# ultravideo/kvazzup

Measured on AMD Instinct MI355X. Metric: hevc_encode_decode_fps, higher is better.
Workload: dtype u8

## Files before the change

### kvazzup_amd/csrc/dec_parse.hip

```cpp
#include <chrono>
#include <cstdio>
#include <cstdlib>
#include <cstring>
#include "decoder.h"

namespace kvzx {

enum { PART_2Nx2N = 0, PART_2NxN, PART_Nx2N, PART_NxN, PART_2NxnU, PART_2NxnD, PART_nLx2N, PART_nRx2N };

namespace {

struct StateTabs { uint8_t next_mps[128], next_lps[128]; uint8_t next[128][2]; uint8_t lps[128][4]; uint32_t lpsn[128][4]; };
const StateTabs &state_tabs()
{
  static const StateTabs t = [] {
    StateTabs t;
    for (int s = 0; s < 128; s++) {
      int st = s >> 1, mps = s & 1;
      t.next_mps[s] = (uint8_t)(((st < 62 ? st + 1 : st) << 1) | mps);
      t.next_lps[s] = (uint8_t)((kNextLps[st] << 1) | (st == 0 ? mps ^ 1 : mps));
      t.next[s][0] = t.next_mps[s]; t.next[s][1] = t.next_lps[s];
      for (int q = 0; q < 4; q++) { t.lps[s][q] = kRangeLps[st][q]; const int n = __builtin_clz((uint32_t)kRangeLps[st][q]) - 23; t.lpsn[s][q] = ((uint32_t)kRangeLps[st][q] << n) | ((uint32_t)n << 16) | ((uint32_t)kRangeLps[st][q] << 24); }
    }
    return t;
  }();
  return t;
}
struct CabacRegs {
  const uint8_t *p = nullptr, *end = nullptr;
  uint64_t value = 0; int bits = 0;
  uint32_t range = 510; uint32_t past = 0;
  const StateTabs *st = nullptr;
  uint16_t *ctx = nullptr;
  static __attribute__((noinline)) uint32_t word_tail(const uint8_t *p, const uint8_t *end) { uint32_t w = 0; for (int i = 0; i < 4; i++) w = (w << 8) | (p + i < end ? p[i] : 0u); return w; }
  __attribute__((always_inline)) inline uint32_t word()
  {
    uint32_t w;
    if (__builtin_expect(p + 4 <= end, 1)) { memcpy(&w, p, 4); w = __builtin_bswap32(w); }
    else { w = word_tail(p, end); past++; }
    p += 4;
    return w;
  }
  __attribute__((always_inline)) inline void refill() { if (__builtin_expect(bits < 16, 0)) { value = (value << 32) | word(); bits += 32; } }
  bool overrun() const { return past > 3; }
  __attribute__((always_inline)) inline int bin(int ci)
  {
    const uint32_t s = ctx[ci];
    const uint32_t e = st->lpsn[s][(range >> 6) & 3];
    const uint32_t rmps = range - (e >> 24);
    const uint64_t scaled = (uint64_t)rmps << bits;
    const bool isl = value >= scaled;
    value -= isl ? scaled : 0;
    const uint32_t nm = (rmps >> 8) ^ 1u;
    range = isl ? (e & 0x1ffu) : (rmps << nm);
    bits -= (int)(isl ? ((e >> 16) & 15u) : nm);
    ctx[ci] = st->next[s][isl];
    refill();
    return (int)((s & 1u) ^ (uint32_t)isl);
  }
  __attribute__((always_inline)) inline int bypass()
  {
    bits--;
    const uint64_t scaled = (uint64_t)range << bits;
    int b = 0;
    if (value >= scaled) { value -= scaled; b = 1; }
    refill();
    return b;
  }
  __attribute__((always_inline)) inline uint32_t bypass_bits(int n)
  {
    uint32_t v = 0;
    while (n > 0) {
      const int m = n > 16 ? 16 : n;
      if (m <= 2) { for (int i = 0; i < m; i++) v = (v << 1) | (uint32_t)bypass(); }
      else {
        bits -= m;
        const uint64_t scaled = (uint64_t)range << bits;
        const uint64_t q = value / scaled;
        value -= q * scaled;
        v = (v << m) | (uint32_t)(q & 0xffffu);
        refill();
      }
      n -= m;
    }
    return v;
  }
  __attribute__((always_inline)) inline int terminate()
  {
    range -= 2;
    if (value >= ((uint64_t)range << bits)) return 1;
    if (range < 256) { range <<= 1; bits--; }
    refill();
    return 0;
  }
};
struct CabacDec : CabacRegs {
  const uint8_t *buf = nullptr;
  uint16_t ctx_store[CTX_COUNT];
  CabacDec() { ctx = ctx_store; }
  CabacDec(const CabacDec &) = delete;
  void load_ctx(const uint8_t *src) { for (int i = 0; i < CTX_COUNT; i++) ctx_store[i] = src[i]; }
  void save_ctx(uint8_t *dst) const { for (int i = 0; i < CTX_COUNT; i++) dst[i] = (uint8_t)ctx_store[i]; }
  void start(const uint8_t *b, size_t l)
  {
    buf = b; p = b; end = b + l; past = 0; st = &state_tabs(); range = 510; ctx = ctx_store;
    value = word(); bits = 32 - 9;
    refill();
  }
  size_t bytes_consumed() const { const size_t consumed_bits = (size_t)(p - buf) * 8 - (size_t)bits; return (consumed_bits + 7) >> 3; }
};

std::atomic<long> g_yields{0};

void parse_sao(CabacDec &c, SaoParams &p, const SaoParams *left, const SaoParams *up, bool luma, bool chroma)
{
  memset(&p, 0, sizeof(p));
  if (left && c.bin(CTX_SAO_MERGE)) { p = *left; return; }
  if (up && c.bin(CTX_SAO_MERGE)) { p = *up; return; }
  for (int ci = 0; ci < 3; ci++) {
    if (!(ci ? chroma : luma)) continue;
    if (ci < 2) p.type[ci] = (uint8_t)(c.bin(CTX_SAO_TYPE) ? (c.bypass() ? 2 : 1) : 0);
    else { p.type[2] = p.type[1]; p.eo_class[2] = p.eo_class[1]; }
    if (!p.type[ci]) continue;
    int a[4];
    for (int i = 0; i < 4; i++) { a[i] = 0; while (a[i] < 7 && c.bypass()) a[i]++; }
    if (p.type[ci] == 1) {
      for (int i = 0; i < 4; i++) if (a[i] && c.bypass()) a[i] = -a[i];
      p.band_pos[ci] = (uint8_t)c.bypass_bits(5);
    } else {
      if (ci < 2) p.eo_class[ci] = (uint8_t)c.bypass_bits(2);
      a[2] = -a[2]; a[3] = -a[3];
    }
    for (int i = 0; i < 4; i++) p.offset[ci][i] = (int8_t)a[i];
  }
}

__attribute__((noinline)) uint32_t sig_flag_run(CabacRegs &cr, const uint8_t *pk, int base, int k0)
{
  CabacRegs c = cr;
  uint32_t sig = 0;
  for (int k = k0; k >= 1; k--) sig |= (uint32_t)c.bin(base + pk[k]) << k;
  cr.p = c.p; cr.value = c.value; cr.bits = c.bits; cr.range = c.range; cr.past = c.past;
  return sig;
}
__attribute__((noinline)) uint32_t greater1_run(CabacRegs &cr, int ctx_base, int n, int *c1_io)
{
  CabacRegs c = cr;
  uint32_t g = 0; int c1 = *c1_io;
  for (int j = 0; j < n; j++) {
    const int g1 = c.bin(ctx_base + c1);
    g |= (uint32_t)g1 << j;
    if (g1) c1 = 0; else if (c1 > 0 && c1 < 3) c1++;
  }
  *c1_io = c1;
  cr.p = c.p; cr.value = c.value; cr.bits = c.bits; cr.range = c.range; cr.past = c.past;
  return g;
}

__attribute__((always_inline)) inline bool parse_residual_regs(CabacRegs &c, int log2, int cidx, int scan_idx, bool sign_hiding, bool ts_enabled, int *tskip, std::vector<uint32_t> &out)
{
  const ScanTabs &S = scan_tabs();
  const int n = 1 << log2, sbl = log2 - 2, nsb = 1 << sbl;
  const uint8_t *SX = S.x[scan_idx][sbl], *SY = S.y[scan_idx][sbl], *PX = S.x[scan_idx][2], *PY = S.y[scan_idx][2];
  uint8_t csbf[8][8]; memset(csbf, 0, sizeof(csbf));
  *tskip = (ts_enabled && log2 == 2) ? c.bin(CTX_TS_FLAG + (cidx ? 1 : 0)) : 0;
  int pre[2];
  for (int d = 0; d < 2; d++) {
    int off, sh, mx = (log2 << 1) - 1, v = 0;
    if (cidx == 0) { off = 3 * (log2 - 2) + ((log2 - 1) >> 2); sh = (log2 + 1) >> 2; } else { off = 15; sh = log2 - 2; }
    while (v < mx && c.bin((d ? CTX_LAST_Y : CTX_LAST_X) + off + (v >> sh))) v++;
    pre[d] = v;
  }
  int lx = pre[0], ly = pre[1];
  if (lx > 3) { int nb = (lx >> 1) - 1; lx = (1 << nb) * (2 + (lx & 1)) + (int)c.bypass_bits(nb); }
  if (ly > 3) { int nb = (ly >> 1) - 1; ly = (1 << nb) * (2 + (ly & 1)) + (int)c.bypass_bits(nb); }
  if (scan_idx == 2) { int tt = lx; lx = ly; ly = tt; }
  if (lx >= n || ly >= n) return false;
  const int last_sb = S.inv[scan_idx][sbl][((ly >> 2) << sbl) | (lx >> 2)], last_pos = S.inv[scan_idx][2][((ly & 3) << 2) | (lx & 3)];
  int c1 = 1;
  for (int i = last_sb; i >= 0; i--) {
    const int xs = SX[i], ys = SY[i];
    int right = (xs < nsb - 1) ? csbf[ys][xs + 1] : 0, below = (ys < nsb - 1) ? csbf[ys + 1][xs] : 0, infer_dc = 0;
    if (i < last_sb && i > 0) { csbf[ys][xs] = (uint8_t)c.bin(CTX_CSBF + ((right | below) ? 1 : 0) + (cidx ? 2 : 0)); infer_dc = 1; }
    else csbf[ys][xs] = 1;
    if (!csbf[ys][xs]) continue;
    uint32_t sig = 0;
    if (i == last_sb) sig |= 1u << last_pos;
    const int prev_csbf = right | (below << 1);
    const uint8_t *pk = S.sigk[scan_idx][log2 == 2 ? 4 : prev_csbf];
    const int sig_base = CTX_SIG + (cidx ? 27 : 0);
    const int sig_off = log2 == 2 ? 0 : (cidx == 0 ? ((i > 0 ? 3 : 0) + ((log2 == 3) ? ((scan_idx == 0) ? 9 : 15) : 21)) : ((log2 == 3) ? 9 : 12));
    {
      const int k0 = (i == last_sb) ? last_pos - 1 : 15;
      const int base = sig_base + sig_off;
      if (k0 >= 1) sig |= sig_flag_run(c, pk, base, k0);
      if (k0 >= 0) {
        if (infer_dc && !(sig >> 1)) sig |= 1u;
        else sig |= (uint32_t)c.bin((i == 0 && log2 != 2) ? sig_base : base + pk[0]);
      }
    }
    if (!sig) continue;
    int ctx_set = (i > 0 && cidx == 0) ? 2 : 0;
    if (c1 == 0) ctx_set++;
    c1 = 1;
    int pos[16], lev[16], nsig = 0, g1idx = -1;
    for (uint32_t m = sig; m;) { const int k = 31 - __builtin_clz(m); pos[nsig++] = k; m &= ~(1u << k); }
    for (int j = 0; j < nsig; j++) lev[j] = 1;
    {
      const uint32_t g = greater1_run(c, CTX_GT1 + (cidx ? 16 : 0) + ctx_set * 4, nsig < 8 ? nsig : 8, &c1);
      if (g) { g1idx = __builtin_ctz(g); for (uint32_t m = g; m; m &= m - 1) lev[__builtin_ctz(m)] = 2; }
    }
    if (g1idx >= 0 && c.bin(CTX_GT2 + (cidx ? 4 : 0) + ctx_set)) lev[g1idx] = 3;
    const bool hidden = sign_hiding && (pos[0] - pos[nsig - 1] > 3);
    const int nsigns = hidden ? nsig - 1 : nsig;
    uint32_t signs = c.bypass_bits(nsigns) << (nsig - nsigns);
    int rice = 0, sum = 0;
    for (int j = 0; j < nsig; j++) {
      int base = (j < 8) ? ((j == g1idx) ? 3 : 2) : 1;
      if (lev[j] == base) {
        int prefix = 0;
        while (prefix < 32 && c.bypass()) prefix++;
        if (prefix - 3 + rice > 16) return false;
        int rem = prefix <= 3 ? (prefix << rice) + (int)c.bypass_bits(rice)
                              : (((1 << (prefix - 3)) + 3 - 1) << rice) + (int)c.bypass_bits(prefix - 3 + rice);
        lev[j] = base + rem;
        if (lev[j] > 3 * (1 << rice)) rice = imin(rice + 1, 4);
      }
      sum += lev[j];
    }
    if (hidden && (sum & 1)) signs |= 1u;
    const size_t o0 = out.size();
    out.resize(o0 + (size_t)nsig);
    uint32_t *dst = out.data() + o0;
    for (int j = 0; j < nsig; j++) {
      const int v = ((signs >> (nsig - 1 - j)) & 1) ? -lev[j] : lev[j];
      const int xp = PX[pos[j]], yp = PY[pos[j]];
      dst[j] = (uint32_t)((((ys << 2) + yp) * n + (xs << 2) + xp) << 16) | ((uint32_t)clip3(-32768, 32767, v) & 0xffffu);
    }
    if (c.overrun()) return false;
  }
  return !c.overrun();
}

bool parse_residual(CabacDec &cd, int log2, int cidx, int scan_idx, bool sign_hiding, bool ts_enabled, int *tskip, std::vector<uint32_t> &out)
{
  CabacRegs c = cd;
  const bool ok = parse_residual_regs(c, log2, cidx, scan_idx, sign_hiding, ts_enabled, tskip, out);
  static_cast<CabacRegs &>(cd) = c;
  return ok;
}

struct MvCand { int mvx, mvy, ref_idx; };

struct SliceParser {
  Decoder::PicJob &job; Decoder::SubOut &out;
  const DecSps &sps; const DecPps &pps; const SliceHdr &sh;
  CabacDec c;
  const int w, h, b4w, b8w, ctbl, mincb, wc, hc;
  B4Rec *b4; uint8_t *pm, *ctd, *im;
  int ref_y0 = -(1 << 30), ref_y1 = 1 << 30;
  int tile_y0 = 0, tile_y1 = 1 << 30, tile_x0 = 0, tile_x1 = 1 << 30;
  const uint8_t *slice_of = nullptr; int cur_slice = 0;
  int slice_qp = 26;
  int err = 0;
  int qp_y = 0, qp_y_pred = 0, last_qp_y = 0, cu_qp_delta_val = 0, log2_qg = 6; bool qp_delta_coded = false;
  int cu_pred_mode = 0, part_mode = 0, max_trafo_depth = 0, intra_modes[4] = {0, 0, 0, 0}, chroma_mode = 0; bool intra_split = false;
  uint32_t ctu_intra_mask = 0;

  SliceParser(Decoder::PicJob &j, Decoder::SubOut &o, int pw)
      : job(j), out(o), sps(*j.sps), pps(j.pps), sh(j.sh), w(j.sps->width), h(j.sps->height), b4w(pw / 4), b8w(pw / 8), ctbl(j.sps->ctb_log2), mincb(j.sps->min_cb_log2), wc(j.sps->wc()),
        hc(j.sps->hc()), b4(j.b4), pm(j.pred_mode.data()), ctd(j.ct_depth.data()), im(j.intra_mode.data())
  { log2_qg = ctbl - pps.qp_delta_depth; }

  inline int bi(int x, int y) const { return (y >> 2) * b4w + (x >> 2); }
  inline int b8(int x, int y) const { return (y >> 3) * b8w + (x >> 3); }
  inline bool avail(int, int, int xn, int yn) const
  {
    return xn >= tile_x0 && yn >= tile_y0 && xn < w && yn < h && yn < tile_y1 && xn < tile_x1 && pm[b8(xn, yn)] != PM_NONE && (!slice_of || slice_of[(yn >> ctbl) * wc + (xn >> ctbl)] == cur_slice);
  }
  void fill_cu8(uint8_t *arr, int x0, int y0, int n, int v)
  {
    const int cols = imin(n, w - x0) >> 3;
    for (int y = y0; y < y0 + n && y < h; y += 8) memset(arr + b8(x0, y), v, (size_t)cols);
  }
  void fill_u8(uint8_t *arr, int x0, int y0, int bw, int bh, int v)
  {
    const int cols = imin(bw, w - x0) >> 2;
    for (int y = y0; y < y0 + bh && y < h; y += 4) memset(arr + bi(x0, y), v, (size_t)cols);
  }
  bool cu_edges_done = false;
  int cu_bypass = 0;
  void fill_recs(int x0, int y0, int bw, int bh, const B4Rec &r, bool cu_edges = false)
  {
    uint64_t v; memcpy(&v, &r, 8);
    const int cols = imin(bw, w - x0) >> 2;
    if (!cu_edges) { for (int y = y0; y < y0 + bh && y < h; y += 4) { uint64_t *p = (uint64_t *)&b4[bi(x0, y)]; for (int i = 0; i < cols; i++) p[i] = v; } return; }
    B4Rec e = r;
    e.flags |= B4_EDGE_V | B4_TU_V; uint64_t vl; memcpy(&vl, &e, 8);
    e.flags = r.flags | B4_EDGE_H | B4_TU_H; uint64_t vt; memcpy(&vt, &e, 8);
    e.flags |= B4_EDGE_V | B4_TU_V; uint64_t vc; memcpy(&vc, &e, 8);
    for (int y = y0; y < y0 + bh && y < h; y += 4) {
      uint64_t *p = (uint64_t *)&b4[bi(x0, y)];
      const bool top = y == y0;
      if (cols > 0) p[0] = top ? vc : vl;
      for (int i = 1; i < cols; i++) p[i] = top ? vt : v;
    }
    cu_edges_done = true;
  }
  void emit_tu(const DecTu &td)
  {
    const int X = td.plane ? td.x * 2 : td.x, Y = td.plane ? td.y * 2 : td.y;
    if (ctbl == 6) {
      TuRange &r = job.region[(Y >> 5) * (b4w >> 3) + (X >> 5)];
      if (!r.count) r.first = (uint32_t)out.tus.size();
      r.count++;
    }
    out.tus.push_back(td);
  }

  bool pb_avail(int xcb, int ycb, int ncbs, int xpb, int ypb, int npbw, int npbh, int part_idx, int xn, int yn) const
  {
    const bool same_cb = xcb <= xn && ycb <= yn && xcb + ncbs > xn && ycb + ncbs > yn;
    bool a;
    if (!same_cb) a = avail(xpb, ypb, xn, yn);
    else a = !((npbw << 1) == ncbs && (npbh << 1) == ncbs && part_idx == 1 && (ycb + npbh <= yn) && (xcb + npbw > xn));
    if (a && pm[b8(xn, yn)] == PM_INTRA) a = false;
    return a;
  }
  static bool same_motion(const B4Rec &a, const B4Rec &b) { return a.ref_idx == b.ref_idx && a.mvx == b.mvx && a.mvy == b.mvy; }

  inline int list_poc(int L, int idx) const { return L ? job.ref_poc1[idx & 15] : job.ref_poc[idx & 15]; }
  inline bool list_lt(int L, int idx) const { return (L ? job.ref_lt1[idx & 15] : job.ref_lt[idx & 15]) != 0; }
  static void scale_by(int &mvx, int &mvy, int td_, int tb_)
  {
    const int td = clip3(-128, 127, td_), tb = clip3(-128, 127, tb_);
    if (td == 0) return;
    const int tx = (16384 + (iabs(td) >> 1)) / td, dsf = clip3(-4096, 4095, (tb * tx + 32) >> 6);
    const int px = dsf * mvx, py = dsf * mvy;
    mvx = clip3(-32768, 32767, (px < 0 ? -1 : 1) * ((iabs(px) + 127) >> 8));
    mvy = clip3(-32768, 32767, (py < 0 ? -1 : 1) * ((iabs(py) + 127) >> 8));
  }
  bool temporal_mv(int xpb, int ypb, int npbw, int npbh, int X, int ref_idx, int &mvx, int &mvy)
  {
    ColMotion *col = job.col.get();
    if (!col) return false;
    const int cy = ypb >> ctbl;
    if (cy < col->hc) {
      std::atomic<uint8_t> &d = col->row_done[(size_t)cy];
      int spins = 0;
      while (!d.load(std::memory_order_acquire)) { if (++spins < 2000) __builtin_ia32_pause(); else std::this_thread::yield(); }
    }
    const int cand[2][2] = {{xpb + npbw, ypb + npbh}, {xpb + (npbw >> 1), ypb + (npbh >> 1)}};
    for (int k = 0; k < 2; k++) {
      int x = cand[k][0], y = cand[k][1];
      if (k == 0 && !((ypb >> ctbl) == (y >> ctbl) && y < h && x < w)) continue;
      x >>= 4; y >>= 4;
      if (x >= col->w16 || y >= col->h16) continue;
      const ColMotion::Mv &m = col->mv[(size_t)y * col->w16 + x];
      if (!m.used) continue;
      const int L = m.used == 2 ? 1 : (m.used == 1 ? 0 : (job.no_backward ? X : sh.collocated_from_l0));
      const bool cur_lt = list_lt(X, ref_idx);
      if ((((m.lt >> L) & 1) != 0) != cur_lt) continue;
      const int col_diff = col->poc - m.ref_poc[L], cur_diff = sh.poc - list_poc(X, ref_idx);
      mvx = m.mv[L][0]; mvy = m.mv[L][1];
      if (!cur_lt && col_diff != cur_diff && col_diff != 0) scale_by(mvx, mvy, col_diff, cur_diff);
      return true;
    }
    return false;
  }

  void merge_candidates(int xcb, int ycb, int ncbs, int xpb, int ypb, int npbw, int npbh, int part_idx, int pmode, MvCand *cand, int want)
  {
    const int lvl = pps.par_mrg_level;
    int n = 0;
    if (lvl > 2 && ncbs == 8) { xpb = xcb; ypb = ycb; npbw = npbh = ncbs; part_idx = 0; pmode = PART_2Nx2N; }
    auto par = [&](int xn, int yn) { return ((xpb >> lvl) == (xn >> lvl)) && ((ypb >> lvl) == (yn >> lvl)); };
    const int xa1 = xpb - 1, ya1 = ypb + npbh - 1, xb1 = xpb + npbw - 1, yb1 = ypb - 1, xb0 = xpb + npbw, yb0 = ypb - 1;
    const int xa0 = xpb - 1, ya0 = ypb + npbh, xb2 = xpb - 1, yb2 = ypb - 1;
    const bool part1 = part_idx == 1;
    const bool nbA1 = pb_avail(xcb, ycb, ncbs, xpb, ypb, npbw, npbh, part_idx, xa1, ya1) && !par(xa1, ya1) &&
                      !(part1 && (pmode == PART_Nx2N || pmode == PART_nLx2N || pmode == PART_nRx2N));
    if (want == 0 && nbA1) { const B4Rec &m = b4[bi(xa1, ya1)]; cand[0].mvx = m.mvx; cand[0].mvy = m.mvy; cand[0].ref_idx = m.ref_idx; return; }
    const bool nbB1 = pb_avail(xcb, ycb, ncbs, xpb, ypb, npbw, npbh, part_idx, xb1, yb1) && !par(xb1, yb1) &&
                      !(part1 && (pmode == PART_2NxN || pmode == PART_2NxnU || pmode == PART_2NxnD));
    const bool nbB0 = pb_avail(xcb, ycb, ncbs, xpb, ypb, npbw, npbh, part_idx, xb0, yb0) && !par(xb0, yb0);
    const bool nbA0 = pb_avail(xcb, ycb, ncbs, xpb, ypb, npbw, npbh, part_idx, xa0, ya0) && !par(xa0, ya0);
    const bool nbB2 = pb_avail(xcb, ycb, ncbs, xpb, ypb, npbw, npbh, part_idx, xb2, yb2) && !par(xb2, yb2);
    const B4Rec zero = B4Rec();
    const B4Rec &A1 = nbA1 ? b4[bi(xa1, ya1)] : zero, &B1 = nbB1 ? b4[bi(xb1, yb1)] : zero, &B0 = nbB0 ? b4[bi(xb0, yb0)] : zero;
    const B4Rec &A0 = nbA0 ? b4[bi(xa0, ya0)] : zero, &B2 = nbB2 ? b4[bi(xb2, yb2)] : zero;
    const bool avA1 = nbA1, avB1 = nbB1 && !(nbA1 && same_motion(A1, B1)), avB0 = nbB0 && !(nbB1 && same_motion(B1, B0));
    const bool avA0 = nbA0 && !(nbA1 && same_motion(A1, A0));
    const bool avB2 = nbB2 && !(nbA1 && same_motion(A1, B2)) && !(nbB1 && same_motion(B1, B2)) && ((int)avA0 + avA1 + avB0 + avB1 != 4);
    const int maxc = sh.max_merge;
    auto add = [&](const B4Rec &m) { if (n < maxc) { cand[n].mvx = m.mvx; cand[n].mvy = m.mvy; cand[n].ref_idx = m.ref_idx; n++; } };
    if (avA1) add(A1);
    if (avB1) add(B1);
    if (avB0) add(B0);
    if (avA0) add(A0);
    if (avB2) add(B2);
    if (n < maxc) { int tx, ty; if (temporal_mv(xpb, ypb, npbw, npbh, 0, 0, tx, ty)) { cand[n].mvx = tx; cand[n].mvy = ty; cand[n].ref_idx = 0; n++; } }
    for (int zi = 0; n < maxc; n++, zi++) { cand[n].mvx = cand[n].mvy = 0; cand[n].ref_idx = zi < sh.num_ref_idx ? zi : 0; }
  }

  void scale_mv(int &mvx, int &mvy, int ref_a, int ref_target) const
  {
    const int td = clip3(-128, 127, sh.poc - job.ref_poc[ref_a]), tb = clip3(-128, 127, sh.poc - job.ref_poc[ref_target]);
    if (td == 0) return;
    const int tx = (16384 + (iabs(td) >> 1)) / td, dsf = clip3(-4096, 4095, (tb * tx + 32) >> 6);
    const int px = dsf * mvx, py = dsf * mvy;
    mvx = clip3(-32768, 32767, (px < 0 ? -1 : 1) * ((iabs(px) + 127) >> 8));
    mvy = clip3(-32768, 32767, (py < 0 ? -1 : 1) * ((iabs(py) + 127) >> 8));
  }

  void amvp_candidates(int xcb, int ycb, int ncbs, int xpb, int ypb, int npbw, int npbh, int part_idx, int ref_idx, int cand[2][2])
  {
    const int xa[2] = {xpb - 1, xpb - 1}, ya[2] = {ypb + npbh, ypb + npbh - 1};
    const int xb[3] = {xpb + npbw, xpb + npbw - 1, xpb - 1}, yb[3] = {ypb - 1, ypb - 1, ypb - 1};
    bool avA[2], avB[3];
    for (int k = 0; k < 2; k++) avA[k] = pb_avail(xcb, ycb, ncbs, xpb, ypb, npbw, npbh, part_idx, xa[k], ya[k]);
    for (int k = 0; k < 3; k++) avB[k] = pb_avail(xcb, ycb, ncbs, xpb, ypb, npbw, npbh, part_idx, xb[k], yb[k]);
    const bool is_scaled = avA[0] || avA[1];
    bool flagA = false, flagB = false; int ax = 0, ay = 0, bx = 0, by = 0;
    const int target = job.ref_poc[ref_idx];
    const bool tlt = job.ref_lt[ref_idx & 15] != 0;
    for (int k = 0; k < 2 && !flagA; k++) if (avA[k]) { const B4Rec &m = b4[bi(xa[k], ya[k])]; if (job.ref_poc[m.ref_idx & 15] == target) { flagA = true; ax = m.mvx; ay = m.mvy; } }
    for (int k = 0; k < 2 && !flagA; k++) if (avA[k]) { const B4Rec &m = b4[bi(xa[k], ya[k])]; if ((job.ref_lt[m.ref_idx & 15] != 0) != tlt) continue; flagA = true; ax = m.mvx; ay = m.mvy; if (!tlt) scale_mv(ax, ay, m.ref_idx & 15, ref_idx); }
    for (int k = 0; k < 3 && !flagB; k++) if (avB[k]) { const B4Rec &m = b4[bi(xb[k], yb[k])]; if (job.ref_poc[m.ref_idx & 15] == target) { flagB = true; bx = m.mvx; by = m.mvy; } }
    if (!is_scaled && flagB) { flagA = true; ax = bx; ay = by; }
    if (!is_scaled) {
      flagB = false;
      for (int k = 0; k < 3 && !flagB; k++) if (avB[k]) {
        const B4Rec &m = b4[bi(xb[k], yb[k])];
        if ((job.ref_lt[m.ref_idx & 15] != 0) != tlt) continue;
        flagB = true; bx = m.mvx; by = m.mvy;
        if (!tlt && job.ref_poc[m.ref_idx & 15] != target) scale_mv(bx, by, m.ref_idx & 15, ref_idx);
      }
    }
    int n = 0;
    if (flagA) { cand[n][0] = ax; cand[n][1] = ay; n++; }
    if (flagB && !(flagA && ax == bx && ay == by)) { cand[n][0] = bx; cand[n][1] = by; n++; }
    if (n < 2) { int tx, ty; if (temporal_mv(xpb, ypb, npbw, npbh, 0, ref_idx, tx, ty)) { cand[n][0] = tx; cand[n][1] = ty; n++; } }
    for (; n < 2; n++) cand[n][0] = cand[n][1] = 0;
  }

  typedef Decoder::PicJob::MvF MvF;
  MvF *mvf = nullptr;
  static bool same_motion_b(const MvF &a, const MvF &b)
  {
    if (a.ref[0] != b.ref[0] || a.ref[1] != b.ref[1]) return false;
    if (a.ref[0] >= 0 && (a.mv[0][0] != b.mv[0][0] || a.mv[0][1] != b.mv[0][1])) return false;
    if (a.ref[1] >= 0 && (a.mv[1][0] != b.mv[1][0] || a.mv[1][1] != b.mv[1][1])) return false;
    return true;
  }
  void merge_candidates_b(int xcb, int ycb, int ncbs, int xpb, int ypb, int npbw, int npbh, int part_idx, int pmode, MvF *cand)
  {
    const int lvl = pps.par_mrg_level;
    int n = 0;
    if (lvl > 2 && ncbs == 8) { xpb = xcb; ypb = ycb; npbw = npbh = ncbs; part_idx = 0; pmode = PART_2Nx2N; }
    auto par = [&](int xn, int yn) { return ((xpb >> lvl) == (xn >> lvl)) && ((ypb >> lvl) == (yn >> lvl)); };
    const int xa1 = xpb - 1, ya1 = ypb + npbh - 1, xb1 = xpb + npbw - 1, yb1 = ypb - 1, xb0 = xpb + npbw, yb0 = ypb - 1;
    const int xa0 = xpb - 1, ya0 = ypb + npbh, xb2 = xpb - 1, yb2 = ypb - 1;
    const bool part1 = part_idx == 1;
    const bool nbA1 = pb_avail(xcb, ycb, ncbs, xpb, ypb, npbw, npbh, part_idx, xa1, ya1) && !par(xa1, ya1) &&
                      !(part1 && (pmode == PART_Nx2N || pmode == PART_nLx2N || pmode == PART_nRx2N));
    const bool nbB1 = pb_avail(xcb, ycb, ncbs, xpb, ypb, npbw, npbh, part_idx, xb1, yb1) && !par(xb1, yb1) &&
                      !(part1 && (pmode == PART_2NxN || pmode == PART_2NxnU || pmode == PART_2NxnD));
    const bool nbB0 = pb_avail(xcb, ycb, ncbs, xpb, ypb, npbw, npbh, part_idx, xb0, yb0) && !par(xb0, yb0);
    const bool nbA0 = pb_avail(xcb, ycb, ncbs, xpb, ypb, npbw, npbh, part_idx, xa0, ya0) && !par(xa0, ya0);
    const bool nbB2 = pb_avail(xcb, ycb, ncbs, xpb, ypb, npbw, npbh, part_idx, xb2, yb2) && !par(xb2, yb2);
    MvF zero; memset(&zero, 0, sizeof(zero)); zero.ref[0] = zero.ref[1] = -1;
    const MvF &A1 = nbA1 ? mvf[bi(xa1, ya1)] : zero, &B1 = nbB1 ? mvf[bi(xb1, yb1)] : zero, &B0 = nbB0 ? mvf[bi(xb0, yb0)] : zero;
    const MvF &A0 = nbA0 ? mvf[bi(xa0, ya0)] : zero, &B2 = nbB2 ? mvf[bi(xb2, yb2)] : zero;
    const bool avA1 = nbA1, avB1 = nbB1 && !(nbA1 && same_motion_b(A1, B1)), avB0 = nbB0 && !(nbB1 && same_motion_b(B1, B0));
    const bool avA0 = nbA0 && !(nbA1 && same_motion_b(A1, A0));
    const bool avB2 = nbB2 && !(nbA1 && same_motion_b(A1, B2)) && !(nbB1 && same_motion_b(B1, B2)) && ((int)avA0 + avA1 + avB0 + avB1 != 4);
    const int maxc = sh.max_merge;
    auto add = [&](const MvF &m) { if (n < maxc) cand[n++] = m; };
    if (avA1) add(A1);
    if (avB1) add(B1);
    if (avB0) add(B0);
    if (avA0) add(A0);
    if (avB2) add(B2);
    if (n < maxc) {
      int x0 = 0, y0 = 0, x1 = 0, y1 = 0;
      const bool f0 = temporal_mv(xpb, ypb, npbw, npbh, 0, 0, x0, y0), f1 = temporal_mv(xpb, ypb, npbw, npbh, 1, 0, x1, y1);
      if (f0 || f1) {
        MvF &t = cand[n++];
        t.mv[0][0] = (int16_t)x0; t.mv[0][1] = (int16_t)y0; t.ref[0] = f0 ? 0 : -1;
        t.mv[1][0] = (int16_t)x1; t.mv[1][1] = (int16_t)y1; t.ref[1] = f1 ? 0 : -1;
      }
    }
    if (n > 1 && n < maxc) {
      static const uint8_t l0c[12] = {0, 1, 0, 2, 1, 2, 0, 3, 1, 3, 2, 3}, l1c[12] = {1, 0, 2, 0, 2, 1, 3, 0, 3, 1, 3, 2};
      const int norig = n;
      for (int comb = 0; comb < norig * (norig - 1) && n < maxc; comb++) {
        const MvF &p0 = cand[l0c[comb]], &p1 = cand[l1c[comb]];
        if (p0.ref[0] < 0 || p1.ref[1] < 0) continue;
        if (list_poc(0, p0.ref[0]) == list_poc(1, p1.ref[1]) && p0.mv[0][0] == p1.mv[1][0] && p0.mv[0][1] == p1.mv[1][1]) continue;
        MvF &t = cand[n++];
        t.mv[0][0] = p0.mv[0][0]; t.mv[0][1] = p0.mv[0][1]; t.ref[0] = p0.ref[0];
        t.mv[1][0] = p1.mv[1][0]; t.mv[1][1] = p1.mv[1][1]; t.ref[1] = p1.ref[1];
      }
    }
    const int nrefs = imin(sh.num_ref_idx, sh.num_ref_idx1);
    for (int zi = 0; n < maxc; n++, zi++) { MvF &t = cand[n]; memset(&t, 0, sizeof(t)); t.ref[0] = t.ref[1] = (int8_t)(zi < nrefs ? zi : 0); }
  }
  void amvp_candidates_b(int xcb, int ycb, int ncbs, int xpb, int ypb, int npbw, int npbh, int part_idx, int X, int ref_idx, int cand[2][2])
  {
    const int xa[2] = {xpb - 1, xpb - 1}, ya[2] = {ypb + npbh, ypb + npbh - 1};
    const int xb[3] = {xpb + npbw, xpb + npbw - 1, xpb - 1}, yb[3] = {ypb - 1, ypb - 1, ypb - 1};
    bool avA[2], avB[3];
    for (int k = 0; k < 2; k++) avA[k] = pb_avail(xcb, ycb, ncbs, xpb, ypb, npbw, npbh, part_idx, xa[k], ya[k]);
    for (int k = 0; k < 3; k++) avB[k] = pb_avail(xcb, ycb, ncbs, xpb, ypb, npbw, npbh, part_idx, xb[k], yb[k]);
    const bool is_scaled = avA[0] || avA[1];
    bool flagA = false, flagB = false; int ax = 0, ay = 0, bx = 0, by = 0;
    const int target = list_poc(X, ref_idx), Y = X ^ 1;
    auto same_pic = [&](const MvF &m, int &vx, int &vy) {
      for (int L : {X, Y}) if (m.ref[L] >= 0 && list_poc(L, m.ref[L]) == target) { vx = m.mv[L][0]; vy = m.mv[L][1]; return true; }
      return false;
    };
    const bool tlt = list_lt(X, ref_idx);
    auto any_pic = [&](const MvF &m, int &vx, int &vy) {
      for (int L : {X, Y}) if (m.ref[L] >= 0 && list_lt(L, m.ref[L]) == tlt) {
        vx = m.mv[L][0]; vy = m.mv[L][1];
        const int poc = list_poc(L, m.ref[L]);
        if (!tlt && poc != target) scale_by(vx, vy, sh.poc - poc, sh.poc - target);
        return true;
      }
      return false;
    };
    for (int k = 0; k < 2 && !flagA; k++) if (avA[k]) flagA = same_pic(mvf[bi(xa[k], ya[k])], ax, ay);
    for (int k = 0; k < 2 && !flagA; k++) if (avA[k]) flagA = any_pic(mvf[bi(xa[k], ya[k])], ax, ay);
    for (int k = 0; k < 3 && !flagB; k++) if (avB[k]) flagB = same_pic(mvf[bi(xb[k], yb[k])], bx, by);
    if (!is_scaled && flagB) { flagA = true; ax = bx; ay = by; }
    if (!is_scaled) {
      flagB = false;
      for (int k = 0; k < 3 && !flagB; k++) if (avB[k]) flagB = any_pic(mvf[bi(xb[k], yb[k])], bx, by);
    }
    int n = 0;
    if (flagA) { cand[n][0] = ax; cand[n][1] = ay; n++; }
    if (flagB && !(flagA && ax == bx && ay == by)) { cand[n][0] = bx; cand[n][1] = by; n++; }
    if (n < 2) { int tx, ty; if (temporal_mv(xpb, ypb, npbw, npbh, X, ref_idx, tx, ty)) { cand[n][0] = tx; cand[n][1] = ty; n++; } }
    for (; n < 2; n++) cand[n][0] = cand[n][1] = 0;
  }
  int parse_ref_idx(int num_active)
  {
    int ref_idx = 0;
    const int mx = num_active - 1;
    while (ref_idx < mx && ref_idx < 2 && c.bin(CTX_REF_IDX + ref_idx)) ref_idx++;
    if (ref_idx == 2) while (ref_idx < mx && c.bypass()) ref_idx++;
    return ref_idx;
// ... 599 lines not shown
```

Baseline: 9577.

## Restructure residual CABAC parsing into per-subblock noinline runs with batched bypass

```diff
diff --git a/kvazzup_amd/csrc/dec_parse.hip b/kvazzup_amd/csrc/dec_parse.hip
--- a/kvazzup_amd/csrc/dec_parse.hip
+++ b/kvazzup_amd/csrc/dec_parse.hip
@@ -84,6 +84,18 @@
       n -= m;
     }
     return v;
+  }
+  __attribute__((always_inline)) inline int bypass_ones()
+  {
+    const uint64_t s16 = (uint64_t)range << (bits - 16);
+    uint64_t q = value / s16;
+    q = q > 0xffffu ? 0xffffu : q;
+    const int ones = __builtin_clz(~((uint32_t)q << 16));
+    const int m = ones < 16 ? ones + 1 : 16;
+    bits -= m;
+    value -= (q >> (16 - m)) * ((uint64_t)range << bits);
+    refill();
+    return ones;
   }
   __attribute__((always_inline)) inline int terminate()
   {
@@ -135,119 +147,144 @@
   }
 }
 
-__attribute__((noinline)) uint32_t sig_flag_run(CabacRegs &cr, const uint8_t *pk, int base, int k0)
+__attribute__((noinline)) uint32_t last_pos_run(CabacRegs &cr, int ts_ctx, int off, int sh, int mx)
 {
   CabacRegs c = cr;
-  uint32_t sig = 0;
-  for (int k = k0; k >= 1; k--) sig |= (uint32_t)c.bin(base + pk[k]) << k;
+  uint32_t r = 0;
+  if (ts_ctx >= 0) r = (uint32_t)c.bin(ts_ctx) << 16;
+  int lx = 0, ly = 0;
+  while (lx < mx && c.bin(CTX_LAST_X + off + (lx >> sh))) lx++;
+  while (ly < mx && c.bin(CTX_LAST_Y + off + (ly >> sh))) ly++;
+  if (lx > 3) { const int nb = (lx >> 1) - 1; lx = (1 << nb) * (2 + (lx & 1)) + (int)c.bypass_bits(nb); }
+  if (ly > 3) { const int nb = (ly >> 1) - 1; ly = (1 << nb) * (2 + (ly & 1)) + (int)c.bypass_bits(nb); }
   cr.p = c.p; cr.value = c.value; cr.bits = c.bits; cr.range = c.range; cr.past = c.past;
-  return sig;
+  return r | ((uint32_t)ly << 8) | (uint32_t)lx;
 }
-__attribute__((noinline)) uint32_t greater1_run(CabacRegs &cr, int ctx_base, int n, int *c1_io)
+struct SbRun {
+  const uint8_t *pk;
+  int csbf_ctx;
+  int sig_ctx, dc_ctx;
+  int k0;
+  uint32_t sig0;
+  int gt1_ctx, gt2_ctx, set0;
+  bool sign_hiding;
+  int c1;
+  uint32_t sig, signs; int nsig; int lev[16];
+};
+enum { SB_NOT_CODED = 0, SB_NO_COEFF = 1, SB_LEVELS = 2, SB_MALFORMED = -1 };
+__attribute__((noinline)) int subblock_run(CabacRegs &cr, SbRun &s)
 {
   CabacRegs c = cr;
-  uint32_t g = 0; int c1 = *c1_io;
-  for (int j = 0; j < n; j++) {
-    const int g1 = c.bin(ctx_base + c1);
-    g |= (uint32_t)g1 << j;
-    if (g1) c1 = 0; else if (c1 > 0 && c1 < 3) c1++;
-  }
-  *c1_io = c1;
-  cr.p = c.p; cr.value = c.value; cr.bits = c.bits; cr.range = c.range; cr.past = c.past;
-  return g;
-}
-
-__attribute__((always_inline)) inline bool parse_residual_regs(CabacRegs &c, int log2, int cidx, int scan_idx, bool sign_hiding, bool ts_enabled, int *tskip, std::vector<uint32_t> &out)
-{
-  const ScanTabs &S = scan_tabs();
-  const int n = 1 << log2, sbl = log2 - 2, nsb = 1 << sbl;
-  const uint8_t *SX = S.x[scan_idx][sbl], *SY = S.y[scan_idx][sbl], *PX = S.x[scan_idx][2], *PY = S.y[scan_idx][2];
-  uint8_t csbf[8][8]; memset(csbf, 0, sizeof(csbf));
-  *tskip = (ts_enabled && log2 == 2) ? c.bin(CTX_TS_FLAG + (cidx ? 1 : 0)) : 0;
-  int pre[2];
-  for (int d = 0; d < 2; d++) {
-    int off, sh, mx = (log2 << 1) - 1, v = 0;
-    if (cidx == 0) { off = 3 * (log2 - 2) + ((log2 - 1) >> 2); sh = (log2 + 1) >> 2; } else { off = 15; sh = log2 - 2; }
-    while (v < mx && c.bin((d ? CTX_LAST_Y : CTX_LAST_X) + off + (v >> sh))) v++;
-    pre[d] = v;
-  }
-  int lx = pre[0], ly = pre[1];
-  if (lx > 3) { int nb = (lx >> 1) - 1; lx = (1 << nb) * (2 + (lx & 1)) + (int)c.bypass_bits(nb); }
-  if (ly > 3) { int nb = (ly >> 1) - 1; ly = (1 << nb) * (2 + (ly & 1)) + (int)c.bypass_bits(nb); }
-  if (scan_idx == 2) { int tt = lx; lx = ly; ly = tt; }
-  if (lx >= n || ly >= n) return false;
-  const int last_sb = S.inv[scan_idx][sbl][((ly >> 2) << sbl) | (lx >> 2)], last_pos = S.inv[scan_idx][2][((ly & 3) << 2) | (lx & 3)];
-  int c1 = 1;
-  for (int i = last_sb; i >= 0; i--) {
-    const int xs = SX[i], ys = SY[i];
-    int right = (xs < nsb - 1) ? csbf[ys][xs + 1] : 0, below = (ys < nsb - 1) ? csbf[ys + 1][xs] : 0, infer_dc = 0;
-    if (i < last_sb && i > 0) { csbf[ys][xs] = (uint8_t)c.bin(CTX_CSBF + ((right | below) ? 1 : 0) + (cidx ? 2 : 0)); infer_dc = 1; }
-    else csbf[ys][xs] = 1;
-    if (!csbf[ys][xs]) continue;
-    uint32_t sig = 0;
-    if (i == last_sb) sig |= 1u << last_pos;
-    const int prev_csbf = right | (below << 1);
-    const uint8_t *pk = S.sigk[scan_idx][log2 == 2 ? 4 : prev_csbf];
-    const int sig_base = CTX_SIG + (cidx ? 27 : 0);
-    const int sig_off = log2 == 2 ? 0 : (cidx == 0 ? ((i > 0 ? 3 : 0) + ((log2 == 3) ? ((scan_idx == 0) ? 9 : 15) : 21)) : ((log2 == 3) ? 9 : 12));
+  int rc = SB_NOT_CODED;
+  do {
+    if (s.csbf_ctx >= 0 && !c.bin(s.csbf_ctx)) break;
+    rc = SB_NO_COEFF;
+    uint32_t sig = s.sig0;
     {
-      const int k0 = (i == last_sb) ? last_pos - 1 : 15;
-      const int base = sig_base + sig_off;
-      if (k0 >= 1) sig |= sig_flag_run(c, pk, base, k0);
+      const uint8_t *const pk = s.pk; const int base = s.sig_ctx, k0 = s.k0;
+      for (int k = k0; k >= 1; k--) sig |= (uint32_t)c.bin(base + pk[k]) << k;
       if (k0 >= 0) {
-        if (infer_dc && !(sig >> 1)) sig |= 1u;
-        else sig |= (uint32_t)c.bin((i == 0 && log2 != 2) ? sig_base : base + pk[0]);
-      }
-    }
-    if (!sig) continue;
-    int ctx_set = (i > 0 && cidx == 0) ? 2 : 0;
-    if (c1 == 0) ctx_set++;
-    c1 = 1;
-    int pos[16], lev[16], nsig = 0, g1idx = -1;
-    for (uint32_t m = sig; m;) { const int k = 31 - __builtin_clz(m); pos[nsig++] = k; m &= ~(1u << k); }
-    for (int j = 0; j < nsig; j++) lev[j] = 1;
+        if (s.csbf_ctx >= 0 && !(sig >> 1)) sig |= 1u;
+        else sig |= (uint32_t)c.bin(s.dc_ctx);
+      }
+    }
+    s.sig = sig;
+    if (!sig) break;
+    rc = SB_LEVELS;
+    const int ctx_set = s.set0 + (s.c1 == 0 ? 1 : 0);
+    const int nsig = __builtin_popcount(sig), n8 = nsig < 8 ? nsig : 8;
+    int *const lev = s.lev;
+    int g1idx = -1;
     {
-      const uint32_t g = greater1_run(c, CTX_GT1 + (cidx ? 16 : 0) + ctx_set * 4, nsig < 8 ? nsig : 8, &c1);
-      if (g) { g1idx = __builtin_ctz(g); for (uint32_t m = g; m; m &= m - 1) lev[__builtin_ctz(m)] = 2; }
-    }
-    if (g1idx >= 0 && c.bin(CTX_GT2 + (cidx ? 4 : 0) + ctx_set)) lev[g1idx] = 3;
-    const bool hidden = sign_hiding && (pos[0] - pos[nsig - 1] > 3);
+      const int g1_ctx = s.gt1_ctx + ctx_set * 4;
+      int c1 = 1; uint32_t g = 0;
+      for (int j = 0; j < n8; j++) {
+        const int g1 = c.bin(g1_ctx + c1);
+        lev[j] = 1 + g1; g |= (uint32_t)g1 << j;
+        if (g1) c1 = 0; else if (c1 > 0 && c1 < 3) c1++;
+      }
+      for (int j = n8; j < nsig; j++) lev[j] = 1;
+      s.c1 = c1;
+      if (g) g1idx = __builtin_ctz(g);
+    }
+    if (g1idx >= 0 && c.bin(s.gt2_ctx + ctx_set)) lev[g1idx] = 3;
+    const bool hidden = s.sign_hiding && ((31 - __builtin_clz(sig)) - __builtin_ctz(sig) > 3);
     const int nsigns = hidden ? nsig - 1 : nsig;
     uint32_t signs = c.bypass_bits(nsigns) << (nsig - nsigns);
     int rice = 0, sum = 0;
     for (int j = 0; j < nsig; j++) {
-      int base = (j < 8) ? ((j == g1idx) ? 3 : 2) : 1;
-      if (lev[j] == base) {
-        int prefix = 0;
-        while (prefix < 32 && c.bypass()) prefix++;
-        if (prefix - 3 + rice > 16) return false;
-        int rem = prefix <= 3 ? (prefix << rice) + (int)c.bypass_bits(rice)
-                              : (((1 << (prefix - 3)) + 3 - 1) << rice) + (int)c.bypass_bits(prefix - 3 + rice);
-        lev[j] = base + rem;
-        if (lev[j] > 3 * (1 << rice)) rice = imin(rice + 1, 4);
-      }
-      sum += lev[j];
+      const int base = (j < 8) ? ((j == g1idx) ? 3 : 2) : 1;
+      int l = lev[j];
+      if (l == base) {
+        int prefix = c.bypass_ones();
+        if (__builtin_expect(prefix == 16, 0)) prefix += c.bypass_ones();
+        if (prefix - 3 + rice > 16) { rc = SB_MALFORMED; break; }
+        const int rem = prefix <= 3 ? (prefix << rice) + (int)c.bypass_bits(rice)
+                                    : (((1 << (prefix - 3)) + 3 - 1) << rice) + (int)c.bypass_bits(prefix - 3 + rice);
+        lev[j] = l = base + rem;
+        if (l > 3 * (1 << rice)) rice = imin(rice + 1, 4);
+      }
+      sum += l;
     }
     if (hidden && (sum & 1)) signs |= 1u;
-    const size_t o0 = out.size();
-    out.resize(o0 + (size_t)nsig);
-    uint32_t *dst = out.data() + o0;
-    for (int j = 0; j < nsig; j++) {
-      const int v = ((signs >> (nsig - 1 - j)) & 1) ? -lev[j] : lev[j];
-      const int xp = PX[pos[j]], yp = PY[pos[j]];
-      dst[j] = (uint32_t)((((ys << 2) + yp) * n + (xs << 2) + xp) << 16) | ((uint32_t)clip3(-32768, 32767, v) & 0xffffu);
-    }
-    if (c.overrun()) return false;
-  }
-  return !c.overrun();
+    s.signs = signs; s.nsig = nsig;
+  } while (0);
+  cr.p = c.p; cr.value = c.value; cr.bits = c.bits; cr.range = c.range; cr.past = c.past;
+  return rc;
 }
 
 bool parse_residual(CabacDec &cd, int log2, int cidx, int scan_idx, bool sign_hiding, bool ts_enabled, int *tskip, std::vector<uint32_t> &out)
 {
-  CabacRegs c = cd;
-  const bool ok = parse_residual_regs(c, log2, cidx, scan_idx, sign_hiding, ts_enabled, tskip, out);
-  static_cast<CabacRegs &>(cd) = c;
-  return ok;
+  CabacRegs &c = cd;
+  const ScanTabs &S = scan_tabs();
+  const int n = 1 << log2, sbl = log2 - 2, nsb = 1 << sbl;
+  const uint8_t *SX = S.x[scan_idx][sbl], *SY = S.y[scan_idx][sbl], *PX = S.x[scan_idx][2], *PY = S.y[scan_idx][2];
+  uint64_t csbf = 0;
+  int lx, ly;
+  {
+    int off, sh;
+    if (cidx == 0) { off = 3 * (log2 - 2) + ((log2 - 1) >> 2); sh = (log2 + 1) >> 2; } else { off = 15; sh = log2 - 2; }
+    const uint32_t r = last_pos_run(c, (ts_enabled && log2 == 2) ? CTX_TS_FLAG + (cidx ? 1 : 0) : -1, off, sh, (log2 << 1) - 1);
+    *tskip = (int)(r >> 16); lx = (int)(r & 0xffu); ly = (int)((r >> 8) & 0xffu);
+  }
+  if (scan_idx == 2) { int tt = lx; lx = ly; ly = tt; }
+  if (lx >= n || ly >= n) return false;
+  const int last_sb = S.inv[scan_idx][sbl][((ly >> 2) << sbl) | (lx >> 2)], last_pos = S.inv[scan_idx][2][((ly & 3) << 2) | (lx & 3)];
+  const size_t o0 = out.size();
+  out.resize(o0 + (size_t)(last_sb * 16 + last_pos + 1));
+  uint32_t *dst = out.data() + o0;
+  SbRun s;
+  s.sign_hiding = sign_hiding; s.c1 = 1;
+  s.gt1_ctx = CTX_GT1 + (cidx ? 16 : 0); s.gt2_ctx = CTX_GT2 + (cidx ? 4 : 0);
+  const int sig_base = CTX_SIG + (cidx ? 27 : 0);
+  for (int i = last_sb; i >= 0; i--) {
+    const int xs = SX[i], ys = SY[i];
+    const int sbit = (ys << 3) | xs;
+    const int right = (xs < nsb - 1) ? (int)((csbf >> (sbit + 1)) & 1) : 0, below = (ys < nsb - 1) ? (int)((csbf >> (sbit + 8)) & 1) : 0;
+    s.csbf_ctx = (i < last_sb && i > 0) ? CTX_CSBF + ((right | below) ? 1 : 0) + (cidx ? 2 : 0) : -1;
+    s.pk = S.sigk[scan_idx][log2 == 2 ? 4 : (right | (below << 1))];
+    s.sig_ctx = sig_base + (log2 == 2 ? 0 : (cidx == 0 ? ((i > 0 ? 3 : 0) + ((log2 == 3) ? ((scan_idx == 0) ? 9 : 15) : 21)) : ((log2 == 3) ? 9 : 12)));
+    s.dc_ctx = (i == 0 && log2 != 2) ? sig_base : s.sig_ctx + s.pk[0];
+    s.k0 = (i == last_sb) ? last_pos - 1 : 15;
+    s.sig0 = (i == last_sb) ? 1u << last_pos : 0u;
+    s.set0 = (i > 0 && cidx == 0) ? 2 : 0;
+    const int rc = subblock_run(c, s);
+    if (rc < 0) { out.resize(o0); return false; }
+    csbf |= (uint64_t)(rc != SB_NOT_CODED) << sbit;
+    if (rc != SB_LEVELS) continue;
+    const int nsig = s.nsig;
+    int j = 0;
+    for (uint32_t m = s.sig; m; j++) {
+      const int k = 31 - __builtin_clz(m); m &= ~(1u << k);
+      const int v = ((s.signs >> (nsig - 1 - j)) & 1) ? -s.lev[j] : s.lev[j];
+      const int xp = PX[k], yp = PY[k];
+      dst[j] = (uint32_t)((((ys << 2) + yp) * n + (xs << 2) + xp) << 16) | ((uint32_t)clip3(-32768, 32767, v) & 0xffffu);
+    }
+    dst += nsig;
+    if (c.overrun()) break;
+  }
+  out.resize((size_t)(dst - out.data()));
+  return !c.overrun();
 }
 
 struct MvCand { int mvx, mvy, ref_idx; };
```

Result: slower. 9353 (-2.3%).
